# snakers4/mnasnet-pytorch

Measured on AMD Instinct MI355X. Metric: images/sec MNASNet-1.0 224^2 bf16 train step, higher is better.
Workload: dtype bf16

## Files before the change

### mnasnet_pytorch_amd/csrc/mnas_dw.hip

```cpp
#include "mnas_common.h"
#ifndef MNAS_DW_XFILL
#define MNAS_DW_XFILL 1
#endif

#ifndef MNAS_DW_NODMA
#define MNAS_DW_NODMA 0
#endif
#ifndef MNAS_DW_NOCOMP
#define MNAS_DW_NOCOMP 0
#endif
#ifndef MNAS_DW_NOBARRIER
#define MNAS_DW_NOBARRIER 0
#endif
__device__ __forceinline__ void dw_step_barrier() {
    if (MNAS_DW_NOBARRIER) asm volatile("s_waitcnt vmcnt(0)" ::: "memory");
    else dma_barrier();
}

#ifndef MNAS_DW_XCD
#define MNAS_DW_XCD 1
#endif
#ifndef MNAS_DW_RA
#define MNAS_DW_RA 1
#endif

#define DW_G 4
#define DW_BW 4
#define DW_RR 8

typedef __attribute__((address_space(3))) void* lds_void_ptr;
typedef const __attribute__((address_space(1))) void* gbl_void_ptr;

struct DwArgs {
    int N, H, W, C;
    int cpw, sx, nthreads, cgn, iw;
    int strips_x, cblocks, items, geff;
    int rc, nb;
    float score;
    int nt;
};

static bool dw_pick(int N, int H, int W, int C, int k, int nrings, int rr, DwArgs* a) {
    const int cps = C / 2;
    int best_sx = 0, best_cpw = 0; double best = -1.0;
    const int maxsx = (W + DW_BW - 1) / DW_BW;
    for (int cpw = 4; cpw <= 128 && cpw <= cps; cpw += 4) {
        if (cps <= 72) { if (cpw != cps) continue; }
        else if (cpw < 32) continue;
        const int cblocks = (cps + cpw - 1) / cpw;
        const int cgn = cpw / 4;
        for (int sx = 1; sx <= maxsx && sx * cpw <= 256; ++sx) {
            const int tw = sx * DW_BW, iw = tw + k - 1;
            size_t lds = (size_t)nrings * rr * iw * cpw * 4;
            const size_t cap = (k == 5 && nrings == 3) ? 60 * 1024 : 78 * 1024;
            if (lds > cap) continue;
            const int nth = ((sx * cpw + 63) / 64) * 64;
            const int rc = iw * cgn;
            if ((rc + 63) / 64 > 2 * (nth / 64)) continue;
            const int strips = (W + tw - 1) / tw;
            const double util = (double)W / (strips * tw) * (double)(sx * cpw) / nth * (double)cps / (cblocks * cpw);
            const double halo = (double)iw / tw;
            const double occ = 0.55 + 0.45 * nth / 256.0;
            const double score = util * occ / (0.6 + 0.4 * halo);
            if (score > best) { best = score; best_sx = sx; best_cpw = cpw; }
        }
    }
    if (best_sx == 0) return false;
    a->score = (float)best;
    const int cpw = best_cpw, cgn = cpw / 4;
    a->N = N; a->H = H; a->W = W; a->C = C;
    a->cpw = cpw; a->sx = best_sx; a->cgn = cgn;
    a->nthreads = ((best_sx * cpw + 63) / 64) * 64;
    a->iw = best_sx * DW_BW + k - 1;
    a->strips_x = (W + best_sx * DW_BW - 1) / (best_sx * DW_BW);
    a->cblocks = (cps + cpw - 1) / cpw;
    a->items = N * a->strips_x * a->cblocks;
    a->rc = a->iw * cgn;
    a->nb = (a->rc + 63) / 64;
    return true;
}

template <int RR>
__device__ __forceinline__ int dw_slot(int image_row) { return (image_row + RR) & (RR - 1); }

__device__ __forceinline__ void dw_item(const DwArgs& a, int item, int& n, int& x0, int& c0) {
    const int cb = item % a.cblocks;
    const int r = item / a.cblocks;
    const int sxi = r % a.strips_x;
    n = r / a.strips_x;
    x0 = sxi * a.sx * DW_BW;
    c0 = cb * 2 * a.cpw;
}

struct DwDma {
    int goff[2];
    bool ok[2];
};

template <int KS>
__device__ __forceinline__ void dw_dma_plan(const DwArgs& a, DwDma& p, int wave, int nwaves, int lane, int x0, int c0) {
    constexpr int PAD = KS / 2;
#pragma unroll
    for (int j = 0; j < 2; ++j) {
        const int b = wave + j * nwaves;
        const int q = b * 64 + lane;
        const int x = q / a.cgn, cgl = q - x * a.cgn;
        const int gx = x0 - PAD + x;
        p.ok[j] = (b < a.nb) && (q < a.rc) && gx >= 0 && gx < a.W && (c0 + cgl * 8) < a.C;
        p.goff[j] = x * (a.C >> 3) + cgl;
    }
}
template <int KS, int G>
__device__ __forceinline__ void dw_dma_rows(const DwArgs& a, const DwDma& p, uint32_t* ring, const uint4* __restrict__ src,
                                            int n, int row0, int x0, int c0, int wave, int nwaves) {
    constexpr int PAD = KS / 2;
    const int C8 = a.C >> 3;
    if (MNAS_DW_NODMA) return;
#pragma unroll
    for (int r = 0; r < G; ++r) {
        const int gy = row0 + r;
        if (gy < 0 || gy >= a.H) continue;
        const uint4* rowsrc = src + ((size_t)n * a.H + gy) * a.W * C8 + (ptrdiff_t)(x0 - PAD) * C8 + (c0 >> 3);
        uint32_t* rowdst = ring + (size_t)dw_slot<2 * G>(gy) * a.rc * 4;
#pragma unroll
        for (int j = 0; j < 2; ++j) {
            const int b = wave + j * nwaves;
            if (b >= a.nb) continue;
            if (p.ok[j])
                __builtin_amdgcn_global_load_lds((gbl_void_ptr)(rowsrc + p.goff[j]), (lds_void_ptr)(rowdst + b * 256), 16, 0, 0);
        }
    }
}

typedef float f2 __attribute__((ext_vector_type(2)));
__device__ __forceinline__ f2 f2fma(f2 a, f2 b, f2 c) { return __builtin_elementwise_fma(a, b, c); }
__device__ __forceinline__ f2 f2bf(uint32_t u) { f2 r; r.x = bf_lo(u); r.y = bf_hi(u); return r; }

template <int WIN_W>
__device__ __forceinline__ void dw_read_act(const uint32_t* rowp, int ps, bool has_coef, f2 s, f2 t, unsigned colmask,
                                            f2 (&xr)[WIN_W]) {
#pragma unroll
    for (int xx = 0; xx < WIN_W; ++xx) {
        f2 v = f2bf(rowp[xx * ps]);
        if (has_coef) {
            v = f2fma(v, s, t);
            v.x = fmaxf(v.x, 0.f); v.y = fmaxf(v.y, 0.f);
        }
        const bool in = (colmask >> xx) & 1u;
        xr[xx].x = in ? v.x : 0.f;
        xr[xx].y = in ? v.y : 0.f;
    }
}

template <int WIN_W>
__device__ __forceinline__ void dw_read_act_nm(const uint32_t* rowp, int ps, bool has_coef, f2 s, f2 t, f2 (&xr)[WIN_W]) {
#pragma unroll
    for (int xx = 0; xx < WIN_W; ++xx) {
        f2 v = f2bf(rowp[xx * ps]);
        if (has_coef) {
            v = f2fma(v, s, t);
            v.x = fmaxf(v.x, 0.f); v.y = fmaxf(v.y, 0.f);
        }
        xr[xx] = v;
    }
}
template <int WIN_W>
__device__ __forceinline__ void dw_ld_raw(const uint32_t* rowp, int ps, uint32_t (&r)[WIN_W]) {
#pragma unroll
    for (int xx = 0; xx < WIN_W; ++xx) r[xx] = rowp[xx * ps];
}
template <int WIN_W>
__device__ __forceinline__ void dw_act_raw(const uint32_t (&r)[WIN_W], bool has_coef, f2 s, f2 t, f2 (&xr)[WIN_W]) {
#pragma unroll
    for (int xx = 0; xx < WIN_W; ++xx) {
        f2 v = f2bf(r[xx]);
        if (has_coef) {
            v = f2fma(v, s, t);
            v.x = fmaxf(v.x, 0.f); v.y = fmaxf(v.y, 0.f);
        }
        xr[xx] = v;
    }
}
template <int RR>
__device__ __forceinline__ void dw_fill_edges(const DwArgs& a, const DwDma& p, uint32_t* ring, int wave, int nwaves, int lane,
                                              bool has_coef) {
    const uint32_t f = has_coef ? 0x7fc07fc0u : 0u;
    const uint4 f4 = make_uint4(f, f, f, f);
#pragma unroll
    for (int j = 0; j < 2; ++j) {
        const int b = wave + j * nwaves, q = b * 64 + lane;
        if (b < a.nb && q < a.rc && !p.ok[j]) {
#pragma unroll
            for (int r = 0; r < RR; ++r) ((uint4*)ring)[(size_t)r * a.rc + q] = f4;
        }
    }
}

template <int WIN_W, bool GM = false>
__device__ __forceinline__ void dw_read_dy(const uint32_t* growp, const uint32_t* yrowp, int ps, const f2 (&cf)[5],
                                           unsigned colmask, f2 (&xr)[WIN_W]) {
#pragma unroll
    for (int xx = 0; xx < WIN_W; ++xx) {
        const f2 g = f2bf(growp[xx * ps]), y = f2bf(yrowp[xx * ps]);
        f2 d;
        f2 dz = g;
        if constexpr (!GM) {
            const f2 z = f2fma(y, cf[0], cf[1]);
            dz.x = (z.x > 0.f) ? g.x : 0.f;
            dz.y = (z.y > 0.f) ? g.y : 0.f;
        }
        d = f2fma(cf[2], dz, f2fma(cf[3], y, cf[4]));
        const bool in = (colmask >> xx) & 1u;
        xr[xx].x = in ? d.x : 0.f;
        xr[xx].y = in ? d.y : 0.f;
    }
}

template <int NV, typename F>
__device__ __forceinline__ void dw_block_reduce(float* scratch, const f2 (&v)[NV], int cp, int sxi, int sx, int cblk,
                                                bool active, F&& emit) {
    __syncthreads();
    if (active) {
#pragma unroll
        for (int k = 0; k < NV; ++k) {
            scratch[(sxi * NV + k) * cblk + 2 * cp] = v[k].x;
            scratch[(sxi * NV + k) * cblk + 2 * cp + 1] = v[k].y;
        }
    }
    __syncthreads();
    for (int i = threadIdx.x; i < NV * cblk; i += blockDim.x) {
        float acc = scratch[i];
        for (int sidx = 1; sidx < sx; ++sidx) acc += scratch[sidx * NV * cblk + i];
        emit(i / cblk, i % cblk, acc);
    }
}

template <int KS, int G, bool HC>
__global__ __launch_bounds__(256, (KS == 3 ? 4 : 3)) void k_dw_fwd(DwArgs a, MnasActIn in, const float* __restrict__ w,
                                                                   const float* __restrict__ bias, uint32_t* __restrict__ out,
                                                                   float* __restrict__ stats) {
    extern __shared__ __attribute__((aligned(16))) unsigned char smem[];
    constexpr int PAD = KS / 2, WIN_W = DW_BW + KS - 1, RR = 2 * G;
    const int cblk = 2 * a.cpw;
    uint32_t* ring = (uint32_t*)smem;
    const int tid = threadIdx.x, lane = tid & 63;
    const int wave = __builtin_amdgcn_readfirstlane(tid >> 6), nwaves = blockDim.x >> 6;
    const int cp = tid % a.cpw, sxi = tid / a.cpw;
    const bool active = sxi < a.sx;
    constexpr bool has_coef = HC;
    const f2 zero2 = {0.f, 0.f};
    f2 s1 = zero2, s2 = zero2;
    int cur_c0 = -1;
    f2 wt[KS * KS], b2 = zero2, cs = {1.f, 1.f}, ct = zero2;
    const int nsteps = (a.H + 2 * PAD + G - 1) / G;
    const int ps = a.cpw;

    const int bid = MNAS_DW_XCD ? (int)xcd_remap(blockIdx.x, a.geff) : (int)blockIdx.x;
    for (int item = bid; item < a.items; item += a.geff) {
        int n, x0, c0;
        dw_item(a, item, n, x0, c0);
        const int ch = c0 + 2 * cp;
        const bool ch_ok = ch < a.C;
        if (c0 != cur_c0) {
            cur_c0 = c0;
#pragma unroll
            for (int t = 0; t < KS * KS; ++t) {
                wt[t].x = ch_ok ? w[(size_t)t * a.C + ch] : 0.f;
                wt[t].y = ch_ok ? w[(size_t)t * a.C + ch + 1] : 0.f;
            }
            b2.x = (bias && ch_ok) ? bias[ch] : 0.f;
            b2.y = (bias && ch_ok) ? bias[ch + 1] : 0.f;
            if (has_coef && ch_ok) { cs.x = in.scale[ch]; cs.y = in.scale[ch + 1]; ct.x = in.shift[ch]; ct.y = in.shift[ch + 1]; }
        }
        DwDma plan;
        dw_dma_plan<KS>(a, plan, wave, nwaves, lane, x0, c0);
        const int gx0 = x0 + sxi * DW_BW;
        f2 A[KS][DW_BW];
#pragma unroll
        for (int i = 0; i < KS; ++i)
#pragma unroll
            for (int j = 0; j < DW_BW; ++j) A[i][j] = b2;
        uint32_t* outp = out + (((size_t)n * a.H * a.W + gx0) * a.C + ch) / 2;
        const uint32_t* colp = ring + (size_t)sxi * DW_BW * ps + cp;

        __syncthreads();
        dw_fill_edges<RR>(a, plan, ring, wave, nwaves, lane, has_coef);
        dw_dma_rows<KS, G>(a, plan, ring, (const uint4*)in.data, n, -PAD, x0, c0, wave, nwaves);
        for (int s = 0; s < nsteps; ++s) {
            const int r0 = -PAD + s * G;
            dw_step_barrier();
            if (s + 1 < nsteps) dw_dma_rows<KS, G>(a, plan, ring, (const uint4*)in.data, n, r0 + G, x0, c0, wave, nwaves);
            if (!active || MNAS_DW_NOCOMP) continue;
            auto row = [&](int iy, const f2 (&xr)[WIN_W], bool have) {
                const int oy = iy - PAD;
                if (have) {
#pragma unroll
                    for (int i = 0; i < KS; ++i)
#pragma unroll
                        for (int ox = 0; ox < DW_BW; ++ox)
#pragma unroll
                            for (int kx = 0; kx < KS; ++kx)
                                A[i][ox] = f2fma(wt[(KS - 1 - i) * KS + kx], xr[ox + kx], A[i][ox]);
                }
                if (oy >= 0 && oy < a.H && ch_ok) {
#pragma unroll
                    for (int ox = 0; ox < DW_BW; ++ox) {
                        if (gx0 + ox < a.W) {
                            const f2 v = A[0][ox];
                            s1 += v;
                            s2 = f2fma(v, v, s2);
                            st_u1(outp + ((size_t)oy * a.W + ox) * a.C / 2, pack_bf16(v.x, v.y), a.nt);
                        }
                    }
                }
#pragma unroll
                for (int i = 0; i + 1 < KS; ++i)
#pragma unroll
                    for (int ox = 0; ox < DW_BW; ++ox) A[i][ox] = A[i + 1][ox];
#pragma unroll
                for (int ox = 0; ox < DW_BW; ++ox) A[KS - 1][ox] = b2;
            };
            const auto rowp = [&](int iy) { return colp + (size_t)dw_slot<RR>(iy) * a.rc * 4; };
            constexpr bool RA = MNAS_DW_RA && KS == 3;
            constexpr int STEP = (KS == 5 && G == 2) ? 1 : 2;
            uint32_t wa[WIN_W], wb[WIN_W];
            if (RA) dw_ld_raw<WIN_W>(rowp(r0), ps, wa);
#pragma unroll (KS == 3 ? G / 2 : 1)
            for (int j = 0; j < G; j += STEP) {
                const int iy = r0 + j;
                const bool in0 = iy >= 0 && iy < a.H, in1 = iy + 1 >= 0 && iy + 1 < a.H;
                f2 xr[WIN_W];
                if constexpr (RA) {
                    dw_ld_raw<WIN_W>(rowp(iy + 1), ps, wb);
                    dw_act_raw<WIN_W>(wa, has_coef, cs, ct, xr);
                    row(iy, xr, in0);
                    if (j + 2 < G) dw_ld_raw<WIN_W>(rowp(iy + 2), ps, wa);
                    dw_act_raw<WIN_W>(wb, has_coef, cs, ct, xr);
                    row(iy + 1, xr, in1);
                } else {
                    if (in0) dw_read_act_nm<WIN_W>(rowp(iy), ps, has_coef, cs, ct, xr);
                    row(iy, xr, in0);
                    if constexpr (STEP == 2) {
                        if (in1) dw_read_act_nm<WIN_W>(rowp(iy + 1), ps, has_coef, cs, ct, xr);
                        row(iy + 1, xr, in1);
                    }
                }
            }
        }
    }
    if (stats) {
        const int rows = a.geff / a.cblocks, col = bid / a.cblocks;
        const int cb0 = (bid % a.cblocks) * cblk;
        const f2 sv[2] = {s1, s2};
        const bool any = cur_c0 >= 0;
        dw_block_reduce<2>((float*)ring, sv, cp, sxi, a.sx, cblk, active, [&](int r, int cl, float v) {
            const int c = cb0 + cl;
            if (c < a.C) stats[((size_t)r * a.C + c) * rows + col] = any ? v : 0.f;
        });
    }
}


template <int KS, bool DG, bool WG, bool RED, int G, bool GM = false, bool HC = true>
__global__ __launch_bounds__(256, ((KS == 5 && DG && (WG || RED)) ? 2 : 3)) void k_dw_bwd(
    DwArgs a, MnasActIn x, MnasGradIn d, const float* __restrict__ w, uint32_t* __restrict__ gin, float* __restrict__ wpartial,
    float* __restrict__ red_partial, const float* __restrict__ red_bn) {
    extern __shared__ __attribute__((aligned(16))) unsigned char smem[];
    constexpr int PAD = KS / 2, WIN_W = DW_BW + KS - 1;
    constexpr bool NEEDX = WG;
    constexpr bool REDG = RED && !WG;
    const int cblk = 2 * a.cpw;
    uint32_t* ring_g = (uint32_t*)smem;
    uint32_t* ring_y = ring_g + (size_t)(2 * G) * a.rc * 4;
    uint32_t* ring_x = ring_y + (size_t)(2 * G) * a.rc * 4;
    const int tid = threadIdx.x, lane = tid & 63;
    const int wave = __builtin_amdgcn_readfirstlane(tid >> 6), nwaves = blockDim.x >> 6;
    const int cp = tid % a.cpw, sxi = tid / a.cpw;
    const bool active = sxi < a.sx;
    constexpr bool has_coef = HC || !WG;
    const uint32_t* xglob = (const uint32_t*)x.data;
    const f2 zero2 = {0.f, 0.f};
    int cur_c0 = -1;
    f2 wt[DG ? KS * KS : 1], wacc[WG ? KS * KS : 1];
    f2 cf[5], cs = {1.f, 1.f}, ct = zero2;
    f2 ris = zero2, rmu = zero2;
    f2 s1 = zero2, s2 = zero2;
#pragma unroll
    for (int t = 0; t < (WG ? KS * KS : 1); ++t) wacc[t] = zero2;
    const int nsteps = (a.H + 2 * PAD + G - 1) / G;
    const int ps = a.cpw;

    const int bid = MNAS_DW_XCD ? (int)xcd_remap(blockIdx.x, a.geff) : (int)blockIdx.x;
    for (int item = bid; item < a.items; item += a.geff) {
        int n, x0, c0;
        dw_item(a, item, n, x0, c0);
        const int ch = c0 + 2 * cp;
        const bool ch_ok = ch < a.C;
        if (c0 != cur_c0) {
            cur_c0 = c0;
            if (DG) {
#pragma unroll
                for (int t = 0; t < KS * KS; ++t) {
                    wt[t].x = ch_ok ? w[(size_t)(KS * KS - 1 - t) * a.C + ch] : 0.f;
                    wt[t].y = ch_ok ? w[(size_t)(KS * KS - 1 - t) * a.C + ch + 1] : 0.f;
                }
            }
#pragma unroll
            for (int r = 0; r < 5; ++r) {
                cf[r].x = ch_ok ? d.coef[(size_t)r * a.C + ch] : 0.f;
                cf[r].y = ch_ok ? d.coef[(size_t)r * a.C + ch + 1] : 0.f;
            }
            if (x.scale != nullptr && ch_ok) { cs.x = x.scale[ch]; cs.y = x.scale[ch + 1]; ct.x = x.shift[ch]; ct.y = x.shift[ch + 1]; }
            if (RED && ch_ok) {
                ris.x = red_bn[6 * a.C + ch]; ris.y = red_bn[6 * a.C + ch + 1];
                rmu.x = -red_bn[5 * a.C + ch] * ris.x; rmu.y = -red_bn[5 * a.C + ch + 1] * ris.y;
            }
        }
        DwDma plan;
        dw_dma_plan<KS>(a, plan, wave, nwaves, lane, x0, c0);
        const int gx0 = x0 + sxi * DW_BW;
        unsigned colmask = 0;
#pragma unroll
        for (int xx = 0; xx < WIN_W; ++xx) { const int gx = gx0 - PAD + xx; colmask |= (gx >= 0 && gx < a.W) ? (1u << xx) : 0u; }
        f2 A[DG ? KS : 1][DW_BW], D[WG ? KS : 1][DW_BW];
#pragma unroll
        for (int i = 0; i < (DG ? KS : 1); ++i)
#pragma unroll
            for (int j = 0; j < DW_BW; ++j) A[i][j] = zero2;
#pragma unroll
        for (int i = 0; i < (WG ? KS : 1); ++i)
#pragma unroll
            for (int j = 0; j < DW_BW; ++j) D[i][j] = zero2;
        const size_t obase = (((size_t)n * a.H * a.W + gx0) * a.C + ch) / 2;
        const size_t coloff = (size_t)sxi * DW_BW * ps + cp;

        auto dma_group = [&](int r0) {
            dw_dma_rows<KS, G>(a, plan, ring_g, (const uint4*)d.g, n, r0, x0, c0, wave, nwaves);
            dw_dma_rows<KS, G>(a, plan, ring_y, (const uint4*)d.y, n, r0, x0, c0, wave, nwaves);
            if (NEEDX) dw_dma_rows<KS, G>(a, plan, ring_x, (const uint4*)x.data, n, r0 - PAD, x0, c0, wave, nwaves);
        };
        uint32_t xq[REDG ? G : 1][DW_BW], xn[REDG ? G : 1][DW_BW];
        auto load_xn = [&](int r0) {
            if constexpr (REDG) {
#pragma unroll
                for (int j = 0; j < G; ++j) {
                    const int oy = r0 - PAD + j;
                    const bool ok = oy >= 0 && oy < a.H && ch_ok && active;
                    const uint32_t* yp = xglob + obase + (size_t)oy * a.W * a.C / 2;
#pragma unroll
                    for (int ox = 0; ox < DW_BW; ++ox) xn[j][ox] = (ok && gx0 + ox < a.W) ? yp[(size_t)ox * a.C / 2] : 0u;
                }
            }
        };
        __syncthreads();
#if MNAS_DW_XFILL
        if (NEEDX) dw_fill_edges<2 * G>(a, plan, ring_x, wave, nwaves, lane, has_coef);
#endif
        dma_group(-PAD);
        load_xn(-PAD);
        for (int s = 0; s < nsteps; ++s) {
            const int r0 = -PAD + s * G;
            dw_step_barrier();
            if constexpr (REDG) {
#pragma unroll
                for (int j = 0; j < G; ++j)
#pragma unroll
                    for (int ox = 0; ox < DW_BW; ++ox) xq[j][ox] = xn[j][ox];
            }
            if (s + 1 < nsteps) { dma_group(r0 + G); load_xn(r0 + G); }
            if (!active || MNAS_DW_NOCOMP) continue;
#pragma unroll 1
            for (int j = 0; j < G; ++j) {
                const int iy = r0 + j;
                const int oy = iy - PAD;
                const bool row_in = iy >= 0 && iy < a.H;
                const bool orow_in = oy >= 0 && oy < a.H;
                uint32_t xraw[DW_BW];
                if constexpr (REDG) {
#pragma unroll
                    for (int ox = 0; ox < DW_BW; ++ox) xraw[ox] = xq[0][ox];
#pragma unroll
                    for (int q = 0; q + 1 < G; ++q)
#pragma unroll
                        for (int ox = 0; ox < DW_BW; ++ox) xq[q][ox] = xq[q + 1][ox];
                }
                f2 xr[WIN_W];
                if (row_in) {
                    const size_t ro = (size_t)dw_slot<2 * G>(iy) * a.rc * 4 + coloff;
                    dw_read_dy<WIN_W, GM>(ring_g + ro, ring_y + ro, ps, cf, colmask, xr);
                } else {
#pragma unroll
                    for (int xx = 0; xx < WIN_W; ++xx) xr[xx] = zero2;
                }
                if (DG && row_in) {
#pragma unroll
                    for (int i = 0; i < KS; ++i)
#pragma unroll
                        for (int ox = 0; ox < DW_BW; ++ox)
#pragma unroll
                            for (int kx = 0; kx < KS; ++kx)
                                A[i][ox] = f2fma(wt[(KS - 1 - i) * KS + kx], xr[ox + kx], A[i][ox]);
                }
                if (WG) {
#pragma unroll
                    for (int q = KS - 1; q > 0; --q)
#pragma unroll
                        for (int ox = 0; ox < DW_BW; ++ox) D[q][ox] = D[q - 1][ox];
#pragma unroll
                    for (int ox = 0; ox < DW_BW; ++ox) D[0][ox] = xr[ox + PAD];
                }
                f2 xa[WIN_W];
                if (NEEDX && orow_in) {
                    const uint32_t* rowp = ring_x + (size_t)dw_slot<2 * G>(oy) * a.rc * 4 + coloff;
#if MNAS_DW_XFILL
                    if (WG) dw_read_act_nm<WIN_W>(rowp, ps, has_coef, cs, ct, xa);
#else
                    if (WG) dw_read_act<WIN_W>(rowp, ps, has_coef, cs, ct, colmask, xa);
#endif
                    if (RED && !REDG) {
#pragma unroll
                        for (int ox = 0; ox < DW_BW; ++ox) xraw[ox] = rowp[(ox + PAD) * ps];
                    }
                }
                if (DG && orow_in && ch_ok) {
#pragma unroll
                    for (int ox = 0; ox < DW_BW; ++ox) {
                        if (gx0 + ox < a.W) {
                            const uint32_t pk = pack_bf16(A[0][ox].x, A[0][ox].y);
                            st_u1(gin + obase + ((size_t)oy * a.W + ox) * a.C / 2, pk, a.nt);
                            if (RED) {
                                const f2 gq = f2bf(pk), yq = f2bf(xraw[ox]);
                                const f2 z = f2fma(yq, cs, ct);
                                f2 dz;
                                dz.x = (z.x > 0.f) ? gq.x : 0.f;
                                dz.y = (z.y > 0.f) ? gq.y : 0.f;
                                s1 += dz;
                                s2 = f2fma(dz, f2fma(yq, ris, rmu), s2);
                            }
                        }
                    }
                }
                if (DG) {
#pragma unroll
                    for (int i = 0; i + 1 < KS; ++i)
#pragma unroll
                        for (int ox = 0; ox < DW_BW; ++ox) A[i][ox] = A[i + 1][ox];
#pragma unroll
                    for (int ox = 0; ox < DW_BW; ++ox) A[KS - 1][ox] = zero2;
                }
                if (WG && orow_in) {
#pragma unroll
                    for (int ky = 0; ky < KS; ++ky)
#pragma unroll
                        for (int ox = 0; ox < DW_BW; ++ox)
#pragma unroll
                            for (int kx = 0; kx < KS; ++kx)
                                wacc[ky * KS + kx] = f2fma(D[ky][ox], xa[ox + kx], wacc[ky * KS + kx]);
                }
            }
        }
    }
    const int row = bid / a.cblocks, rows = a.geff / a.cblocks;
    const int cb0 = (bid % a.cblocks) * cblk;
    const bool any = cur_c0 >= 0;
    if constexpr (RED) {
        const f2 sv[2] = {s1, s2};
        dw_block_reduce<2>((float*)ring_g, sv, cp, sxi, a.sx, cblk, active, [&](int r, int cl, float v) {
            const int c = cb0 + cl;
            if (c < a.C) red_partial[((size_t)r * a.C + c) * rows + row] = any ? v : 0.f;
        });
    }
    if constexpr (WG) {
        dw_block_reduce<KS * KS>((float*)ring_g, wacc, cp, sxi, a.sx, cblk, active, [&](int k, int cl, float v) {
            const int c = cb0 + cl;
            if (c < a.C) wpartial[((size_t)row * KS * KS + k) * a.C + c] = any ? v : 0.f;
        });
    }
}

static int dw_rings(int form) { return form < 0 ? 1 : (form == 1 ? 2 : 3); }
static bool dw_force(int N, int H, int W, int C, int k, int nrings, DwArgs* a, int* g) {
    const int cpw = mnas_diag_env("MNAS_DW_CPW", 0), sx = mnas_diag_env("MNAS_DW_SX", 0), gg = mnas_diag_env("MNAS_DW_G", 0);
    if (cpw <= 0 || sx <= 0 || (gg != 2 && gg != 4) || (cpw & 3) || cpw * sx > 256 || cpw > C / 2) return false;
    const int cps = C / 2, cgn = cpw / 4, iw = sx * DW_BW + k - 1;
    if ((size_t)nrings * 2 * gg * iw * cpw * 4 > 160 * 1024) return false;
    a->N = N; a->H = H; a->W = W; a->C = C; a->score = 0.f;
    a->cpw = cpw; a->sx = sx; a->cgn = cgn;
    a->nthreads = ((sx * cpw + 63) / 64) * 64;
    a->iw = iw;
    a->strips_x = (W + sx * DW_BW - 1) / (sx * DW_BW);
    a->cblocks = (cps + cpw - 1) / cpw;
    a->items = N * a->strips_x * a->cblocks;
    a->rc = iw * cgn;
    a->nb = (a->rc + 63) / 64;
    if (a->nb > 2 * (a->nthreads / 64)) return false;
    *g = gg;
    return true;
}
static bool dw_choose(int N, int H, int W, int C, int k, int form, DwArgs* a, int* g) {
    DwArgs a4, a2;
    const int nrings = dw_rings(form);
    if (mnas_diag_env("MNAS_DW_CPW", 0) > 0 && dw_force(N, H, W, C, k, nrings, a, g)) return true;
    const bool ok4 = dw_pick(N, H, W, C, k, nrings, 8, &a4), ok2 = dw_pick(N, H, W, C, k, nrings, 4, &a2);
    if (!ok4 && !ok2) return false;
    if (ok2 && (!ok4 || 0.93f * a2.score > a4.score)) { *a = a2; *g = 2; }
    else { *a = a4; *g = 4; }
    return true;
}
static bool dw_finish(DwArgs* a, int nparts) {
    if (nparts < a->cblocks) return false;
    int g = nparts < a->items ? nparts : a->items;
    a->geff = g / a->cblocks * a->cblocks;
    return a->geff >= a->cblocks;
}
static const int dw_form_of[4] = {-1, 0, 1, 2};
extern "C" int mnas_dw_rows(int N, int H, int W, int C, int k, int nparts, int which) {
    if (which == 4 || which == 7) return mnas_dw2_rows(N, H, W, C, k, nparts, which - 4);
    if (which < 0 || which > 3) return -1;
    DwArgs a;
    int g;
    if (!dw_choose(N, H, W, C, k, dw_form_of[which], &a, &g) || !dw_finish(&a, nparts)) return -1;
    return a.geff / a.cblocks;
}

extern "C" int mnas_dw_geometry(int N, int H, int W, int C, int k, int which, int* out) {
    if (which < 0 || which > 3 || !out) return MNAS_EINVAL;
    DwArgs a;
    int g;
    if (!dw_choose(N, H, W, C, k, dw_form_of[which], &a, &g)) return MNAS_EINVAL;
    out[0] = a.cpw; out[1] = a.sx; out[2] = a.nthreads; out[3] = a.strips_x; out[4] = a.cblocks;
    out[5] = dw_rings(dw_form_of[which]) * 2 * g * a.rc * 16; out[6] = g;
    return MNAS_OK;
}

extern "C" int mnas_dw_fwd(const MnasDwFwd* c, void* stream) {
    if (!c || (c->k != 3 && c->k != 5) || (c->C & 7) || c->nparts < 1 || c->stride < 0 || c->stride > 2) return MNAS_EINVAL;
    if (c->stride == 2) return mnas_dw2_fwd(c, stream);
    DwArgs a;
    int g;
    if (!dw_choose(c->N, c->H, c->W, c->C, c->k, -1, &a, &g) || !dw_finish(&a, c->nparts)) return MNAS_EINVAL;
    a.nt = (mnas_nt_mask() & MNAS_NT_DW_FWD) ? 1 : 0;
    size_t lds = (size_t)2 * g * a.rc * 16;
    const size_t red_need = (size_t)a.sx * 2 * 2 * a.cpw * sizeof(float);
    if (lds < red_need) lds = red_need;
    hipStream_t s = (hipStream_t)stream;
#define MNAS_DWF(K_, G_) do { if (c->in.scale) hipLaunchKernelGGL((k_dw_fwd<K_, G_, true>), dim3(a.geff), dim3(a.nthreads), lds, s, a, c->in, c->w, c->bias, \
                                            (uint32_t*)c->out, c->stats); \
                              else hipLaunchKernelGGL((k_dw_fwd<K_, G_, false>), dim3(a.geff), dim3(a.nthreads), lds, s, a, c->in, c->w, c->bias, \
                                            (uint32_t*)c->out, c->stats); } while (0)
    if (c->k == 3) { if (g == 4) MNAS_DWF(3, 4); else MNAS_DWF(3, 2); }
    else { if (g == 4) MNAS_DWF(5, 4); else MNAS_DWF(5, 2); }
#undef MNAS_DWF
    MNAS_CHECK_LAUNCH();
    return MNAS_OK;
}

template <int KS, bool DG, bool WG, bool RED, int G, bool GM>
static void dw_bwd_launch(const DwArgs& a, size_t lds, hipStream_t s, const MnasDwBwd* c) {
    if constexpr (WG) {
        if (!c->x.scale) {
            hipLaunchKernelGGL((k_dw_bwd<KS, DG, WG, RED, G, GM, false>), dim3(a.geff), dim3(a.nthreads), lds, s, a, c->x, c->dy, c->w,
                               (uint32_t*)c->gin, c->wpartial, c->red_partial, c->red_bn);
            return;
        }
    }
    hipLaunchKernelGGL((k_dw_bwd<KS, DG, WG, RED, G, GM, true>), dim3(a.geff), dim3(a.nthreads), lds, s, a, c->x, c->dy, c->w,
                       (uint32_t*)c->gin, c->wpartial, c->red_partial, c->red_bn);
}

extern "C" int mnas_dw_bwd(const MnasDwBwd* c, void* stream) {
    if (!c || (c->k != 3 && c->k != 5) || (c->C & 7) || c->nparts < 1 || c->phase < 0 || c->phase > 2) return MNAS_EINVAL;
    if (c->stride < 0 || c->stride > 2) return MNAS_EINVAL;
    if (c->stride == 2) return mnas_dw2_bwd(c, stream);
    hipStream_t s = (hipStream_t)stream;
    if (!c->x.data || !c->dy.g) return MNAS_EINVAL;
    const bool red = c->red_bn != nullptr && c->red_partial != nullptr;
    const bool want_dg = c->phase != 2, want_wg = c->phase != 1;
    const int nrings = dw_rings(c->phase);
    DwArgs a;
    int g;
    if (!dw_choose(c->N, c->H, c->W, c->C, c->k, c->phase, &a, &g) || !dw_finish(&a, c->nparts)) return MNAS_EINVAL;
    a.nt = (mnas_nt_mask() & MNAS_NT_DW_BWD) ? 1 : 0;
    size_t lds = (size_t)nrings * 2 * g * a.rc * 16;
    const size_t red_need = (size_t)a.sx * (want_wg ? c->k * c->k : 2) * 2 * a.cpw * sizeof(float);
    if (lds < red_need) lds = red_need;
#define MNAS_DWB(K_, DG_, WG_, R_, G_) dw_bwd_launch<K_, DG_, WG_, R_, G_, false>(a, lds, s, c)
#define MNAS_DWB_G(K_, DG_, WG_, R_) do { if (g == 4) MNAS_DWB(K_, DG_, WG_, R_, 4); else MNAS_DWB(K_, DG_, WG_, R_, 2); } while (0)
    if (c->g_masked) {
        if (!(want_dg && want_wg && red)) return MNAS_EINVAL;
        if (c->k == 3) { if (g == 4) dw_bwd_launch<3, true, true, true, 4, true>(a, lds, s, c); else dw_bwd_launch<3, true, true, true, 2, true>(a, lds, s, c); }
        else { if (g == 4) dw_bwd_launch<5, true, true, true, 4, true>(a, lds, s, c); else dw_bwd_launch<5, true, true, true, 2, true>(a, lds, s, c); }
        MNAS_CHECK_LAUNCH();
        return MNAS_OK;
    }
    if (c->k == 3) {
        if (want_dg && want_wg) { if (red) MNAS_DWB_G(3, true, true, true); else MNAS_DWB_G(3, true, true, false); }
        else if (want_dg) { if (red) MNAS_DWB_G(3, true, false, true); else MNAS_DWB_G(3, true, false, false); }
        else MNAS_DWB_G(3, false, true, false);
    } else {
        if (want_dg && want_wg) { if (red) MNAS_DWB_G(5, true, true, true); else MNAS_DWB_G(5, true, true, false); }
        else if (want_dg) { if (red) MNAS_DWB_G(5, true, false, true); else MNAS_DWB_G(5, true, false, false); }
        else MNAS_DWB_G(5, false, true, false);
    }
#undef MNAS_DWB_G
#undef MNAS_DWB
    MNAS_CHECK_LAUNCH();
    return MNAS_OK;
}
```

Before: 26220.

## Unroll depthwise row loop by kernel size to rotate accumulators statically

Replaces the per-row shift of the accumulator array A and the dy history D with a modular rotation indexed by a compile-time row phase, unrolling the row loop by KS via a static_for helper. DMA group barriers are folded into the unrolled row sequence. This applies to the forward KS==5 path and the backward path. It aims to remove the register-to-register moves spent shifting the rolling windows, at the cost of larger code and more register pressure from the KS-way unroll.

```diff
diff --git a/mnasnet_pytorch_amd/csrc/mnas_dw.hip b/mnasnet_pytorch_amd/csrc/mnas_dw.hip
--- a/mnasnet_pytorch_amd/csrc/mnas_dw.hip
+++ b/mnasnet_pytorch_amd/csrc/mnas_dw.hip
@@ -1,4 +1,5 @@
 #include "mnas_common.h"
+#include <type_traits>
 #ifndef MNAS_DW_XFILL
 #define MNAS_DW_XFILL 1
 #endif
@@ -136,6 +137,13 @@
 __device__ __forceinline__ f2 f2fma(f2 a, f2 b, f2 c) { return __builtin_elementwise_fma(a, b, c); }
 __device__ __forceinline__ f2 f2bf(uint32_t u) { f2 r; r.x = bf_lo(u); r.y = bf_hi(u); return r; }
 
+template <int I, int N, typename F>
+__device__ __forceinline__ void dw_static_for_(F& f) {
+    if constexpr (I < N) { f(std::integral_constant<int, I>()); dw_static_for_<I + 1, N>(f); }
+}
+template <int N, typename F>
+__device__ __forceinline__ void dw_static_for(F&& f) { dw_static_for_<0, N>(f); }
+
 template <int WIN_W>
 __device__ __forceinline__ void dw_read_act(const uint32_t* rowp, int ps, bool has_coef, f2 s, f2 t, unsigned colmask,
                                             f2 (&xr)[WIN_W]) {
@@ -286,6 +294,53 @@
         __syncthreads();
         dw_fill_edges<RR>(a, plan, ring, wave, nwaves, lane, has_coef);
         dw_dma_rows<KS, G>(a, plan, ring, (const uint4*)in.data, n, -PAD, x0, c0, wave, nwaves);
+        if constexpr (KS == 5) {
+            const int T = nsteps * G;
+            auto row = [&](auto U, int t) __attribute__((always_inline)) {
+                constexpr int u = decltype(U)::value;
+                if ((t & (G - 1)) == 0) {
+                    int s = t / G, r0 = t - PAD;
+                    asm volatile("; dw group" : "+s"(s), "+s"(r0));
+                    dw_step_barrier();
+                    if (s + 1 < nsteps) dw_dma_rows<KS, G>(a, plan, ring, (const uint4*)in.data, n, r0 + G, x0, c0, wave, nwaves);
+                    asm volatile("; dw group end");
+                }
+                if (!active || MNAS_DW_NOCOMP) return;
+                const int iy = t - PAD, oy = iy - PAD;
+                if (iy >= 0 && iy < a.H) {
+                    f2 xr[WIN_W];
+                    dw_read_act_nm<WIN_W>(colp + (size_t)dw_slot<RR>(iy) * a.rc * 4, ps, has_coef, cs, ct, xr);
+#pragma unroll
+                    for (int i = 0; i < KS; ++i)
+#pragma unroll
+                        for (int ox = 0; ox < DW_BW; ++ox)
+#pragma unroll
+                            for (int kx = 0; kx < KS; ++kx)
+                                A[(i + u) % KS][ox] = f2fma(wt[(KS - 1 - i) * KS + kx], xr[ox + kx], A[(i + u) % KS][ox]);
+                }
+                if (oy >= 0 && oy < a.H && ch_ok) {
+#pragma unroll
+                    for (int ox = 0; ox < DW_BW; ++ox) {
+                        if (gx0 + ox < a.W) {
+                            const f2 v = A[u][ox];
+                            s1 += v;
+                            s2 = f2fma(v, v, s2);
+                            st_u1(outp + ((size_t)oy * a.W + ox) * a.C / 2, pack_bf16(v.x, v.y), a.nt);
+                        }
+                    }
+                }
+#pragma unroll
+                for (int ox = 0; ox < DW_BW; ++ox) A[u][ox] = b2;
+            };
+#pragma unroll 1
+            for (int t0 = 0; t0 < T; t0 += KS) {
+                dw_static_for<KS>([&](auto U) __attribute__((always_inline)) {
+                    const int t = t0 + decltype(U)::value;
+                    if (t < T) row(U, t);
+                });
+            }
+            continue;
+        }
         for (int s = 0; s < nsteps; ++s) {
             const int r0 = -PAD + s * G;
             dw_step_barrier();
@@ -458,106 +513,108 @@
 #endif
         dma_group(-PAD);
         load_xn(-PAD);
-        for (int s = 0; s < nsteps; ++s) {
-            const int r0 = -PAD + s * G;
-            dw_step_barrier();
+        const int T = nsteps * G;
+        auto row = [&](auto U, int t) {
+            constexpr int u = decltype(U)::value;
+            if ((t & (G - 1)) == 0) {
+                int s = t / G, r0 = t - PAD;
+                asm volatile("; dw group" : "+s"(s), "+s"(r0));
+                dw_step_barrier();
+                if constexpr (REDG) {
+#pragma unroll
+                    for (int j = 0; j < G; ++j)
+#pragma unroll
+                        for (int ox = 0; ox < DW_BW; ++ox) xq[j][ox] = xn[j][ox];
+                }
+                if (s + 1 < nsteps) { dma_group(r0 + G); load_xn(r0 + G); }
+                asm volatile("; dw group end");
+            }
+            if (!active || MNAS_DW_NOCOMP) return;
+            const int iy = t - PAD;
+            const int oy = iy - PAD;
+            const bool row_in = iy >= 0 && iy < a.H;
+            const bool orow_in = oy >= 0 && oy < a.H;
+            uint32_t xraw[DW_BW];
             if constexpr (REDG) {
 #pragma unroll
-                for (int j = 0; j < G; ++j)
-#pragma unroll
-                    for (int ox = 0; ox < DW_BW; ++ox) xq[j][ox] = xn[j][ox];
-            }
-            if (s + 1 < nsteps) { dma_group(r0 + G); load_xn(r0 + G); }
-            if (!active || MNAS_DW_NOCOMP) continue;
-#pragma unroll 1
-            for (int j = 0; j < G; ++j) {
-                const int iy = r0 + j;
-                const int oy = iy - PAD;
-                const bool row_in = iy >= 0 && iy < a.H;
-                const bool orow_in = oy >= 0 && oy < a.H;
-                uint32_t xraw[DW_BW];
-                if constexpr (REDG) {
-#pragma unroll
-                    for (int ox = 0; ox < DW_BW; ++ox) xraw[ox] = xq[0][ox];
-#pragma unroll
-                    for (int q = 0; q + 1 < G; ++q)
-#pragma unroll
-                        for (int ox = 0; ox < DW_BW; ++ox) xq[q][ox] = xq[q + 1][ox];
-                }
-                f2 xr[WIN_W];
-                if (row_in) {
-                    const size_t ro = (size_t)dw_slot<2 * G>(iy) * a.rc * 4 + coloff;
-                    dw_read_dy<WIN_W, GM>(ring_g + ro, ring_y + ro, ps, cf, colmask, xr);
-                } else {
-#pragma unroll
-                    for (int xx = 0; xx < WIN_W; ++xx) xr[xx] = zero2;
-                }
-                if (DG && row_in) {
-#pragma unroll
-                    for (int i = 0; i < KS; ++i)
-#pragma unroll
-                        for (int ox = 0; ox < DW_BW; ++ox)
-#pragma unroll
-                            for (int kx = 0; kx < KS; ++kx)
-                                A[i][ox] = f2fma(wt[(KS - 1 - i) * KS + kx], xr[ox + kx], A[i][ox]);
-                }
-                if (WG) {
-#pragma unroll
-                    for (int q = KS - 1; q > 0; --q)
-#pragma unroll
-                        for (int ox = 0; ox < DW_BW; ++ox) D[q][ox] = D[q - 1][ox];
-#pragma unroll
-                    for (int ox = 0; ox < DW_BW; ++ox) D[0][ox] = xr[ox + PAD];
-                }
-                f2 xa[WIN_W];
-                if (NEEDX && orow_in) {
-                    const uint32_t* rowp = ring_x + (size_t)dw_slot<2 * G>(oy) * a.rc * 4 + coloff;
+                for (int ox = 0; ox < DW_BW; ++ox) xraw[ox] = xq[0][ox];
+#pragma unroll
+                for (int q = 0; q + 1 < G; ++q)
+#pragma unroll
+                    for (int ox = 0; ox < DW_BW; ++ox) xq[q][ox] = xq[q + 1][ox];
+            }
+            f2 xr[WIN_W];
+            if (row_in) {
+                const size_t ro = (size_t)dw_slot<2 * G>(iy) * a.rc * 4 + coloff;
+                dw_read_dy<WIN_W, GM>(ring_g + ro, ring_y + ro, ps, cf, colmask, xr);
+            } else {
+#pragma unroll
+                for (int xx = 0; xx < WIN_W; ++xx) xr[xx] = zero2;
+            }
+            if (DG && row_in) {
+#pragma unroll
+                for (int i = 0; i < KS; ++i)
+#pragma unroll
+                    for (int ox = 0; ox < DW_BW; ++ox)
+#pragma unroll
+                        for (int kx = 0; kx < KS; ++kx)
+                            A[(i + u) % KS][ox] = f2fma(wt[(KS - 1 - i) * KS + kx], xr[ox + kx], A[(i + u) % KS][ox]);
+            }
+            if (WG) {
+#pragma unroll
+                for (int ox = 0; ox < DW_BW; ++ox) D[u][ox] = xr[ox + PAD];
+            }
+            f2 xa[WIN_W];
+            if (NEEDX && orow_in) {
+                const uint32_t* rowp = ring_x + (size_t)dw_slot<2 * G>(oy) * a.rc * 4 + coloff;
 #if MNAS_DW_XFILL
-                    if (WG) dw_read_act_nm<WIN_W>(rowp, ps, has_coef, cs, ct, xa);
+                if (WG) dw_read_act_nm<WIN_W>(rowp, ps, has_coef, cs, ct, xa);
 #else
-                    if (WG) dw_read_act<WIN_W>(rowp, ps, has_coef, cs, ct, colmask, xa);
+                if (WG) dw_read_act<WIN_W>(rowp, ps, has_coef, cs, ct, colmask, xa);
 #endif
-                    if (RED && !REDG) {
-#pragma unroll
-                        for (int ox = 0; ox < DW_BW; ++ox) xraw[ox] = rowp[(ox + PAD) * ps];
-                    }
-                }
-                if (DG && orow_in && ch_ok) {
-#pragma unroll
-                    for (int ox = 0; ox < DW_BW; ++ox) {
-                        if (gx0 + ox < a.W) {
-                            const uint32_t pk = pack_bf16(A[0][ox].x, A[0][ox].y);
-                            st_u1(gin + obase + ((size_t)oy * a.W + ox) * a.C / 2, pk, a.nt);
-                            if (RED) {
-                                const f2 gq = f2bf(pk), yq = f2bf(xraw[ox]);
-                                const f2 z = f2fma(yq, cs, ct);
-                                f2 dz;
-                                dz.x = (z.x > 0.f) ? gq.x : 0.f;
-                                dz.y = (z.y > 0.f) ? gq.y : 0.f;
-                                s1 += dz;
-                                s2 = f2fma(dz, f2fma(yq, ris, rmu), s2);
-                            }
+                if (RED && !REDG) {
+#pragma unroll
+                    for (int ox = 0; ox < DW_BW; ++ox) xraw[ox] = rowp[(ox + PAD) * ps];
+                }
+            }
+            if (DG && orow_in && ch_ok) {
+#pragma unroll
+                for (int ox = 0; ox < DW_BW; ++ox) {
+                    if (gx0 + ox < a.W) {
+                        const uint32_t pk = pack_bf16(A[u][ox].x, A[u][ox].y);
+                        st_u1(gin + obase + ((size_t)oy * a.W + ox) * a.C / 2, pk, a.nt);
+                        if (RED) {
+                            const f2 gq = f2bf(pk), yq = f2bf(xraw[ox]);
+                            const f2 z = f2fma(yq, cs, ct);
+                            f2 dz;
+                            dz.x = (z.x > 0.f) ? gq.x : 0.f;
+                            dz.y = (z.y > 0.f) ? gq.y : 0.f;
+                            s1 += dz;
+                            s2 = f2fma(dz, f2fma(yq, ris, rmu), s2);
                         }
                     }
                 }
-                if (DG) {
-#pragma unroll
-                    for (int i = 0; i + 1 < KS; ++i)
-#pragma unroll
-                        for (int ox = 0; ox < DW_BW; ++ox) A[i][ox] = A[i + 1][ox];
-#pragma unroll
-                    for (int ox = 0; ox < DW_BW; ++ox) A[KS - 1][ox] = zero2;
-                }
-                if (WG && orow_in) {
-#pragma unroll
-                    for (int ky = 0; ky < KS; ++ky)
-#pragma unroll
-                        for (int ox = 0; ox < DW_BW; ++ox)
-#pragma unroll
-                            for (int kx = 0; kx < KS; ++kx)
-                                wacc[ky * KS + kx] = f2fma(D[ky][ox], xa[ox + kx], wacc[ky * KS + kx]);
-                }
-            }
+            }
+            if (DG) {
+#pragma unroll
+                for (int ox = 0; ox < DW_BW; ++ox) A[u][ox] = zero2;
+            }
+            if (WG && orow_in) {
+#pragma unroll
+                for (int ky = 0; ky < KS; ++ky)
+#pragma unroll
+                    for (int ox = 0; ox < DW_BW; ++ox)
+#pragma unroll
+                        for (int kx = 0; kx < KS; ++kx)
+                            wacc[ky * KS + kx] = f2fma(D[(u - ky + KS) % KS][ox], xa[ox + kx], wacc[ky * KS + kx]);
+            }
+        };
+#pragma unroll 1
+        for (int t0 = 0; t0 < T; t0 += KS) {
+            dw_static_for<KS>([&](auto U) {
+                const int t = t0 + decltype(U)::value;
+                if (t < T) row(U, t);
+            });
         }
     }
     const int row = bid / a.cblocks, rows = a.geff / a.cblocks;
```

Result: no change. 26330, median of 6 (+0.4%).
